# seung-lab/euclidean-distance-transform-3d

Hardware: AMD Instinct MI355X
Metric: Mvox/s edt3dsq 512^3 uint32 (higher is better)
Workload: dtype u16 integer quanta (exact) with f64 envelope fallback / f32 storage / u32 labels; 1 GPU; cfg2: 512^3 uint32 labels, anisotropy (6.0, 6.0, 30.0), black_border=True, device-resident in/out

## Files before the change

### euclidean-distance-transform-3d_amd/csrc/edt_api.hip

```cpp
#include <algorithm>
#include <atomic>
#include <cstdlib>
#include <cstring>
#include <mutex>
#include <system_error>
#include <thread>
#include <vector>

#include <sys/mman.h>

#include "edt_common.h"
#include "edt_kernels.h"

#include "edt_api_internal.h"

namespace edt_amd {

static thread_local std::string g_last_error = "";
#ifdef EDT_DIAG
constexpr int kDiagMask = ~0;
#else
constexpr int kDiagMask = kDiagFormBits;
#endif
static int env_debug_mode() {
// ... 32 lines not shown


struct Plan {
  int ndim;
  int64_t sx, sy, sz, voxels;
  AxisGeom gy, gz;
  float *bufB = nullptr;
  int32_t *stack = nullptr;
  uint32_t *nz_y = nullptr, *rs_y = nullptr, *zs_y = nullptr, *nz_z = nullptr, *rs_z = nullptr;
  unsigned char *line_ws = nullptr;
  uint16_t *codes = nullptr;
  int64_t xy_slab = 0;
  bool codes_whole = false;
  int64_t code_pitch = 0;
  uint32_t *q16_counts = nullptr, *q16_ids = nullptr;
  uint32_t *q16_map = nullptr;
  int q16_map_words = 0;
  int64_t q16_id_capacity = 0;
  size_t bytes = 0;
};

AxisGeom make_geom_y(int64_t sx, int64_t sy, int64_t sz) {
  AxisGeom g;
  g.sx = sx; g.n = sy; g.stride = sx; g.nouter = sz; g.outer_stride = sx * sy;
  g.nbands = ceil_div(sy, kBandRows);
  return g;
}
AxisGeom make_geom_z(int64_t sx, int64_t sy, int64_t sz) {
  AxisGeom g;
  g.sx = sx; g.n = sz; g.stride = sx * sy; g.nouter = sy; g.outer_stride = sx;
  g.nbands = ceil_div(sz, kBandRows);
  return g;
}

static bool plan_needs_pingpong(int ndim, int64_t sx, int64_t sy, int64_t sz, int flags);

constexpr int64_t kCodeSlabVoxels = (int64_t)1 << 27;
static int64_t whole_index_limit() {
  static const int64_t v = [] {
    const char *e = std::getenv("EDT_HIP_WHOLE_INDEX_BYTES");
    return e ? (int64_t)std::strtoll(e, nullptr, 0) : (int64_t)8 << 30;
  }();
  return v;
}
static int64_t plane_pad_elems(int64_t sx, int64_t sy) {
  const char *e = std::getenv("EDT_HIP_PLANE_PAD_BYTES");
  const int64_t forced = (e && *e) ? (int64_t)std::strtoll(e, nullptr, 0) : (int64_t)-1;
  if (forced >= 0) return (forced & ~(int64_t)7) / 2;
  const int64_t slice = sx * sy * (int64_t)sizeof(uint16_t);
  if (slice % ((int64_t)2 << 20) == 0) return 8192 / 2;
  if (slice % ((int64_t)1 << 20) == 0) return 4096 / 2;
  return 0;
}
constexpr int kQ16Slots = 256;
constexpr int EDT_FLAG_NO_INDEX_FORM = 0x8000;
static int64_t plan_code_slab(int dtype, int ndim, int64_t sx, int64_t sy, int64_t sz, int flags) {
  if (ndim < 2 || sx % 4 != 0 || sx * sy > kCodeSlabVoxels || (flags & (EDT_FLAG_NO_INDEX_FORM | EDT_FLAG_SMALL_WORKSPACE))) return 0;
  if ((flags & EDT_FLAG_FORCE_GENERIC) || env_force_generic() || (g_debug_mode & (0x100000 | 64 | 32))) return 0;
  if (!row_pass_wave_supported(dtype, sx, sy, sz) || !column_pass_wave_supported(make_geom_y(sx, sy, sz))) return 0;
  int64_t slab = kCodeSlabVoxels / (sx * sy);
  if (slab >= sz) return sz;
  if (slab >= 32) slab &= ~(int64_t)31;
  return slab;
}

static Plan make_plan(int dtype, int ndim, int64_t sx, int64_t sy, int64_t sz, void *ws, int flags) {
  Plan p;
  p.ndim = ndim; p.sx = sx; p.sy = sy; p.sz = sz; p.voxels = sx * sy * sz;
  p.gy = make_geom_y(sx, sy, sz);
  p.gz = make_geom_z(sx, sy, sz);
  Carver c(ws);
  if (ndim >= 2) {
    if (plan_needs_pingpong(ndim, sx, sy, sz, flags)) {
      p.bufB = c.take<float>((size_t)p.voxels);
      p.stack = c.take<int32_t>((size_t)p.voxels);
    }
    const size_t wy = (size_t)(p.gy.sx * p.gy.nbands * p.gy.nouter);
    p.nz_y = c.take<uint32_t>(wy);
    p.rs_y = c.take<uint32_t>(wy);
  }
  if (ndim >= 3 && !(flags & EDT_FLAG_BATCH_2D)) {
    const size_t wy = (size_t)(p.gy.sx * p.gy.nbands * p.gy.nouter);
    const size_t wz = (size_t)(p.gz.sx * p.gz.nbands * p.gz.nouter);
    p.nz_z = c.take<uint32_t>(wz);
    if (wz <= wy) p.rs_z = p.rs_y;
    else p.rs_z = c.take<uint32_t>(wz);
    p.zs_y = c.take<uint32_t>(wy);
  }
  if (ndim >= 2) {
    p.xy_slab = plan_code_slab(dtype, ndim, sx, sy, sz, flags);
    p.codes_whole = p.xy_slab >= sz || (p.xy_slab > 0 && p.xy_slab % 32 == 0 && ndim == 3 && !(flags & EDT_FLAG_BATCH_2D) &&
                                        sx * sy * sz * (int64_t)sizeof(uint16_t) <= whole_index_limit());
    p.code_pitch = sx * sy + ((p.codes_whole && ndim == 3 && sz > 1 && !(flags & EDT_FLAG_BATCH_2D)) ? plane_pad_elems(sx, sy) : 0);
    if (p.xy_slab > 0) p.codes = c.take<uint16_t>((size_t)((p.codes_whole ? sz : p.xy_slab) * p.code_pitch));
  }
  if (ndim >= 2 && !(flags & EDT_FLAG_FORCE_GENERIC) && !env_force_generic()) {
    const int64_t ty = ceil_div(sx, 16) * (ceil_div(sz, 8) * 8);
    const int64_t tz = ceil_div(sx, 16) * (ceil_div(sy, 8) * 8);
    p.q16_map_words = (int)ceil_div(sz, 32);
    p.q16_counts = c.take<uint32_t>(kQ16Slots + (size_t)(ceil_div(sx, 32) * p.q16_map_words));
    p.q16_map = p.q16_counts ? p.q16_counts + kQ16Slots : nullptr;
    p.q16_id_capacity = std::max(ty, tz);
    p.q16_ids = c.take<uint32_t>((size_t)p.q16_id_capacity);
  }
  if (ndim == 1) (void)c.take<unsigned char>(line_workspace_bytes(sx));
  if (ndim >= 2 && !row_pass_tiled_supported(sx) && !row_pass_wave_supported(dtype, sx, sy, sz) &&
      !(flags & EDT_FLAG_FORCE_GENERIC) && !env_force_generic())
    p.line_ws = c.take<unsigned char>(rows_line_workspace_bytes(sx, sy * sz));
  p.bytes = align_up(c.off, 256) + 256;
  return p;
}

bool column_inplace_supported(const AxisGeom &g) {
  return column_pass_wave_supported(g) || column_pass_tiled_supported(g);
}
int launch_column_inplace(float *F, const uint32_t *nz, const uint32_t *rs, const AxisGeom &g,
// ... 75 lines not shown
                      float wx, float wy, float wz, int flags, float *d_out, void *d_ws,
                      size_t ws_bytes, hipStream_t stream) {
  int rc = check_shape(dtype, ndim, sx, sy, sz);
  if (rc != EDT_OK) return rc;
  if ((rc = check_voxel_sizes(ndim, wx, wy, wz)) != EDT_OK) return rc;
  if (sx == 0 || sy == 0 || sz == 0) return EDT_OK;
  if (!d_labels || !d_out) { set_error("null device pointer"); return EDT_ERR_BAD_ARG; }
  Plan p = make_plan(dtype, ndim, sx, sy, sz, d_ws, flags);
  if (d_ws && ws_bytes < p.bytes && p.codes != nullptr) p = make_plan(dtype, ndim, sx, sy, sz, d_ws, flags | EDT_FLAG_NO_INDEX_FORM);
  const bool line_without_ws = ndim == 1 && (!d_ws || ws_bytes < p.bytes);
  if (!line_without_ws && (!d_ws || ws_bytes < p.bytes)) {
    set_error("workspace too small: need " + std::to_string(p.bytes) +
              " bytes (edt_hip_workspace_bytes_flags with the flags of this call)");
    return EDT_ERR_BAD_ARG;
  }
  const int bb = (flags & EDT_FLAG_BLACK_BORDER) ? 1 : 0;
  const int want_sqrt = (flags & EDT_FLAG_SQRT) ? 1 : 0;
  const int signed_tf = (flags & EDT_FLAG_SIGNED) ? 1 : 0;
  if (signed_tf && !signed_transform_supported(dtype, ndim, sx, sy, sz, flags)) {
    set_error("EDT_FLAG_SIGNED: shape not served by the one-transform form (edt_hip_signed_supported)");
    return EDT_ERR_UNSUPPORTED;
  }
  const int last_epi = (bb ? 0 : kEpiToInf) | (want_sqrt ? kEpiSqrt : 0) | kEpiStream;
  if ((flags & EDT_FLAG_BATCH_2D) && ndim != 3) { set_error("EDT_FLAG_BATCH_2D needs ndim = 3 (sz = image count)"); return EDT_ERR_BAD_ARG; }
  const bool zpass = ndim == 3 && !(flags & EDT_FLAG_BATCH_2D);
  const bool binary_yz = (flags & EDT_FLAG_BINARY_YZ) != 0 && dtype != EDT_BOOL;
  const float fmin_y = edt_hip_field_floor(wx, wx);
  const float fmin_z = edt_hip_field_floor(wx, wy);
  p.gy.fmin = fmin_y;
  p.gz.fmin = fmin_z;

  if (g_log.enabled.load(std::memory_order_relaxed)) {
    std::lock_guard<std::mutex> lock(g_log_mutex);
    log_begin_call();
  }

  float q16_q = 1.0f;
  uint32_t q16_a[3] = {1u, 1u, 1u};
  bool q16 = false;
  int q16_slot = 0;
  bool q16_counts_zeroed = false;
  if (ndim >= 2 && p.q16_counts != nullptr) {
    const float ws3[3] = {wx, wy, wz};
    q16 = q16_quantum(ws3, (ndim == 3 && !(flags & EDT_FLAG_BATCH_2D)) ? 3 : 2, &q16_q, q16_a);
  }
  constexpr int kQ16Off = 16 | 64 | 0x2000 | 0x4000 | 0x8000 | 0x10000;
  auto q16_cannot_refuse = [&](int axis, const AxisGeom &g) {
    return q16 && q16_no_refusals(q16_q, q16_a, axis, sx, sy, g.n, bb);
  };
  auto q16_applies = [&](const AxisGeom &g) {
    return q16 && column_pass_q16_supported(g) && column_pass_wave_supported(g) && !(g_debug_mode & kQ16Off) &&
           ceil_div(g.sx, 16) * (ceil_div(g.nouter, 8) * 8) <= p.q16_id_capacity;
  };
  auto q16_pass = [&](float *F, const uint16_t *codes, const uint32_t *rs, const AxisGeom &g, int axis, int epi,
                      TileList &list, uint16_t *plane, bool sure, bool &launched, int64_t map_words_off = 0,
                      const uint32_t *signbits = nullptr) -> int {
    list = TileList();
    launched = false;
    if (!q16 || q16_slot >= kQ16Slots || !column_pass_q16_supported(g) || !column_pass_wave_supported(g) ||
        !column_pass_q16_aligned(F, codes, plane) || (g_debug_mode & kQ16Off))
      return EDT_OK;
    if (ceil_div(g.sx, 16) * (ceil_div(g.nouter, 8) * 8) > p.q16_id_capacity) return EDT_OK;
    sure = sure && q16_cannot_refuse(axis, g);
    if (!sure && !q16_counts_zeroed) {
      EDT_HIP_TRY(hipMemsetAsync(p.q16_counts, 0, kQ16Slots * sizeof(uint32_t), stream));
      q16_counts_zeroed = true;
    }
    uint32_t *count = p.q16_counts + q16_slot++;
    const bool reads_plane = codes == nullptr && plane != nullptr;
    const int r = launch_column_pass_q16(F, codes, rs, g, q16_q, q16_a[axis], q16_a[0], bb, epi, count, p.q16_ids, stream,
                                         nullptr, plane, p.q16_map + map_words_off, p.q16_map_words, nullptr,
                                         reads_plane ? p.code_pitch : 0, reads_plane ? sx : 0,
                                         (axis == 1 && plane != nullptr && codes != nullptr && q16_value_limit(q16_q, q16_a[2], sz, bb) != 0u) ? 1 : 0,
                                         signbits, (codes != nullptr && axis == 1) ? p.code_pitch : 0);
    if (r != EDT_OK) return r;
    launched = true;
    list.count = count;
    list.ids = p.q16_ids;
    list.none = sure;
    return EDT_OK;
  };

  if (ndim == 1) {
    ScopedPass t("x_pass", stream);
    if (force_generic_1d(flags) || line_without_ws) return launch_row_pass_serial(dtype, d_labels, d_out, sx, 1, wx, bb, 0, want_sqrt, stream);
    return launch_line_pass(dtype, d_labels, d_out, sx, wx, bb, want_sqrt, d_ws, stream);
  }

  const bool force_generic = (flags & EDT_FLAG_FORCE_GENERIC) != 0 || env_force_generic();
  const bool tiled_y = !force_generic && column_inplace_supported(p.gy);
  const bool tiled_z = !force_generic && column_inplace_supported(p.gz);
  const int swaps = (tiled_y ? 0 : 1) + ((zpass && !tiled_z) ? 1 : 0);
  float *cur = (swaps % 2 == 0) ? d_out : p.bufB;
  float *other = (cur == d_out) ? p.bufB : d_out;
  const bool tiled_x = !force_generic && (row_pass_tiled_supported(sx) || row_pass_wave_supported(dtype, sx, sy, sz));
  const bool index_form = p.codes != nullptr && tiled_x && tiled_y && row_codes_exact(wx, sx);
  bool plane16 = q16 && index_form && zpass && p.codes_whole && !(g_debug_mode & (kQ16Off | 0x10000000)) &&
                       column_pass_q16_supported(p.gy) && column_pass_q16_supported(p.gz) &&
                       column_pass_wave_supported(p.gy) && column_pass_wave_supported(p.gz);
  bool y_sure = true;
  const bool q16_only = zpass && index_form && tiled_z && q16_applies(p.gy) && q16_applies(p.gz) && q16_cannot_refuse(1, p.gy) &&
                        q16_cannot_refuse(2, p.gz) && column_pass_q16_aligned(cur, p.codes, p.codes) &&
                        ceil_div(sz, p.xy_slab > 0 ? p.xy_slab : sz) + 1 <= kQ16Slots;
  const bool fuse_sign = signed_tf && q16_only && !(g_debug_mode & 0x400);
  const int zero_label = fuse_sign ? 2 : signed_tf;
  const bool skip_nz = q16_only && !signed_tf && !binary_yz && !(g_debug_mode & 0x400);
  uint32_t *const nzy = skip_nz ? nullptr : p.nz_y, *const nzz = skip_nz ? nullptr : p.nz_z;
  if (index_form) {
    const int64_t sxy = sx * sy, wpl = p.gy.sx * p.gy.nbands;
    const size_t lsz = dtype_size(dtype);
    const bool one = p.xy_slab >= sz;
    ScopedPass whole(one ? nullptr : "xy_pass", stream);
    for (int64_t z0 = 0; z0 < sz; z0 += p.xy_slab) {
      const int64_t zc = std::min<int64_t>(p.xy_slab, sz - z0);
      const char *lab = static_cast<const char *>(d_labels) + (size_t)(z0 * sxy) * lsz;
      uint16_t *slab_codes = p.codes + ((p.codes_whole && !one) ? z0 * p.code_pitch : 0);
      {
        ScopedPass t(one ? "x_pass" : nullptr, stream);
        rc = launch_row_pass_wave(dtype, lab, nullptr, nzy ? nzy + z0 * wpl : nullptr, p.rs_y + z0 * wpl,
                                  zpass ? p.zs_y + z0 * wpl : nullptr, sx, sy, zc, wx, bb, bb ? 0 : 1, stream,
                                  z0 > 0 ? lab - (size_t)sxy * lsz : nullptr, slab_codes, zero_label, p.code_pitch);
        if (rc != EDT_OK) return rc;
        if (binary_yz) {
          AxisGeom gb = p.gy;
          gb.nouter = zc;
          rc = launch_planes_one_run(p.nz_y + z0 * wpl, p.rs_y + z0 * wpl, zpass ? p.zs_y + z0 * wpl : nullptr, gb, z0, stream);
          if (rc != EDT_OK) return rc;
        }
      }
      {
        ScopedPass t(one ? "y_pass" : nullptr, stream);
        AxisGeom g = p.gy;
        g.nouter = zc;
        TileList list;
        bool launched = false;
        rc = q16_pass(cur + z0 * sxy, slab_codes, p.rs_y + z0 * wpl, g, 1, zpass ? 0 : last_epi, list, plane16 ? slab_codes : nullptr,
                      true, launched, (p.codes_whole && !one) ? z0 / 32 : 0);
        if (rc != EDT_OK) return rc;
        if (!launched) plane16 = false;
        y_sure = y_sure && list.none;
        if (q16_only && (!launched || !list.none)) { set_error("internal: pass Y left the integer kernel"); return EDT_ERR_HIP; }
        if (!list.none)
          rc = launch_column_pass_wave_codes(cur + z0 * sxy, slab_codes, p.nz_y + z0 * wpl, p.rs_y + z0 * wpl, g, wy, bb,
                                             zpass ? 0 : last_epi, wx, bb ? 0 : 1, stream, nullptr, list, ColumnOut(), p.code_pitch);
        if (rc != EDT_OK) return rc;
      }
    }
  } else if (tiled_x) {
    {
      ScopedPass t("x_pass", stream);
      if (signed_tf)
        rc = launch_row_pass_wave(dtype, d_labels, cur, p.nz_y, p.rs_y, zpass ? p.zs_y : nullptr, sx, sy, sz, wx, bb, bb ? 0 : 1,
                                  stream, nullptr, nullptr, 1);
      else
        rc = launch_row_bits(dtype, d_labels, cur, p.nz_y, p.rs_y, zpass ? p.zs_y : nullptr, sx, sy, sz,
                             wx, bb, bb ? 0 : 1, stream);
      if (rc != EDT_OK) return rc;
      if (binary_yz) rc = launch_planes_one_run(p.nz_y, p.rs_y, zpass ? p.zs_y : nullptr, p.gy, 0, stream);
      if (rc != EDT_OK) return rc;
    }
  } else {
    {
      ScopedPass t("x_pass", stream);
      if (p.line_ws != nullptr) rc = launch_rows_line_pass(dtype, d_labels, cur, sx, sy * sz, wx, bb, bb ? 0 : 1, p.line_ws, stream);
      else rc = launch_row_pass_serial(dtype, d_labels, cur, sx, sy * sz, wx, bb, bb ? 0 : 1, 0, stream);
      if (rc != EDT_OK) return rc;
    }
    {
      ScopedPass t("y_bits", stream);
      rc = launch_axis_bits(dtype, d_labels, nullptr, p.nz_y, p.rs_y, p.gy, stream);
      if (rc != EDT_OK) return rc;
      if (binary_yz) rc = launch_planes_one_run(p.nz_y, p.rs_y, nullptr, p.gy, 0, stream);
      if (rc != EDT_OK) return rc;
    }
  }
  if (!index_form) {
    ScopedPass t("y_pass", stream);
    const int epi = zpass ? 0 : last_epi;
    if (tiled_y) {
      TileList list;
      bool launched = false;
      rc = q16_pass(cur, nullptr, p.rs_y, p.gy, 1, epi, list, nullptr, false, launched);
      if (rc != EDT_OK) return rc;
      y_sure = false;
      rc = launch_column_inplace(cur, p.nz_y, p.rs_y, p.gy, wy, bb, epi, stream, list);
    } else {
      rc = launch_column_pass_serial(cur, other, p.nz_y, p.rs_y, p.stack, p.gy, wy, bb, epi, stream);
      std::swap(cur, other);
    }
    if (rc != EDT_OK) return rc;
  }
  if (zpass) {
    ScopedPass t("z_bits", stream);
    if (tiled_x) rc = launch_bits_transpose_yz(nzy, p.zs_y, nzz, p.rs_z, sx, sy, sz, stream);
    else {
      rc = launch_axis_bits(dtype, d_labels, nullptr, p.nz_z, p.rs_z, p.gz, stream);
      if (rc == EDT_OK && binary_yz) rc = launch_planes_one_run(p.nz_z, p.rs_z, nullptr, p.gz, 0, stream);
    }
// ... 50 lines not shown
  }
  return n;
}

const char *edt_hip_last_error(void) { return last_error_cstr(); }

int edt_hip_index_form_exact(float wx, int64_t sx) { return (sx >= 1 && row_codes_exact(wx, sx)) ? 1 : 0; }

const char *edt_hip_version(void) { return "edt_hip 0.1 (gfx950)"; }

size_t edt_hip_workspace_bytes_flags(int dtype, int ndim, int64_t sx, int64_t sy, int64_t sz, int flags) {
  if (check_shape(dtype, ndim, sx, sy, sz) != EDT_OK) return 0;
  if (sx == 0 || sy == 0 || sz == 0) return 256;
  return make_plan(dtype, ndim, sx, sy, sz, nullptr, flags).bytes;
}

int edt_hip_signed_supported(int dtype, int ndim, int64_t sx, int64_t sy, int64_t sz, int flags) {
  if (check_shape(dtype, ndim, sx, sy, sz) != EDT_OK) return 0;
  return signed_transform_supported(dtype, ndim, sx, sy, sz, flags) ? 1 : 0;
}

size_t edt_hip_workspace_bytes(int dtype, int ndim, int64_t sx, int64_t sy, int64_t sz) {
  return edt_hip_workspace_bytes_flags(dtype, ndim, sx, sy, sz, 0);
}

int edt_hip_edtsq_device(const void *d_labels, int dtype, int ndim, int64_t sx, int64_t sy,
                         int64_t sz, float wx, float wy, float wz, int flags, float *d_output,
                         void *d_workspace, size_t workspace_bytes, void *stream) {
  return run_device(d_labels, dtype, ndim, sx, sy, sz, wx, wy, wz, flags, d_output, d_workspace,
                    workspace_bytes, (hipStream_t)stream);
}

int edt_hip_set_debug_mode(int mode) {
  set_thread_debug_mode(mode);
  return EDT_OK;
}

int edt_hip_get_debug_mode(void) { return debug_mode(); }

int edt_hip_q16_no_refusals(int64_t sx, int64_t sy, int64_t sz, float wx, float wy, float wz, int ndim, int black_border,
                            int *pass_y, int *pass_z) {
  if (pass_y) *pass_y = 0;
  if (pass_z) *pass_z = 0;
  if (ndim < 2 || ndim > 3 || sx < 1 || sy < 1 || (ndim == 3 && sz < 1)) return 0;
  const float w3[3] = {wx, wy, wz};
  float q = 1.0f;
  uint32_t a[3] = {1u, 1u, 1u};
  if (!q16_quantum(w3, ndim, &q, a)) return 0;
  const bool y = q16_no_refusals(q, a, 1, sx, sy, sy, black_border);
  const bool z = ndim == 3 && y && q16_no_refusals(q, a, 2, sx, sy, sz, black_border);
  if (pass_y) *pass_y = y ? 1 : 0;
  if (pass_z) *pass_z = z ? 1 : 0;
  return 1;
}

int edt_hip_set_profiling(int enabled) {
  std::lock_guard<std::mutex> lock(g_log_mutex);
  g_log.enabled.store(enabled != 0);
  log_begin_call();
  return EDT_OK;
}

int edt_hip_get_pass_times(float *ms, int capacity) {
  std::lock_guard<std::mutex> lock(g_log_mutex);
  int n = (int)g_log.span.size();
  for (int i = 0; i < n && i < capacity; ++i) {
    float t = 0.0f;
    if (hipEventElapsedTime(&t, g_log.pool[g_log.span[i].first], g_log.pool[g_log.span[i].second]) !=
        hipSuccess) {
      (void)hipGetLastError();
      t = -1.0f;
    }
    ms[i] = t;
  }
  return n;
}

const char *edt_hip_get_pass_name(int index) {
  std::lock_guard<std::mutex> lock(g_log_mutex);
  if (index < 0 || index >= (int)g_log.names.size()) return "";
  return g_log.names[index].c_str();
}

float edt_hip_field_floor(float wx, float wy) {
  const float a = wx * wx, b = wy * wy;
  if (!(a > 0.0f) || !(b > 0.0f) || !(a < INFINITY) || !(b < INFINITY)) return 0.0f;
  return a < b ? a : b;
}

int edt_hip_subtract_device(const float *d_a, const float *d_b, float *d_out, int64_t count,
                            void *stream) {
  return launch_subtract(d_a, d_b, d_out, count, (hipStream_t)stream);
}

static bool vg_use_native(int ndim, int64_t sx, int64_t sy, int64_t sz) {
  return !(g_debug_mode & 0x20000) && vg_native_supported(ndim, sx, sy, sz);
}

size_t edt_hip_voxel_graph_workspace_bytes(int ndim, int64_t sx, int64_t sy, int64_t sz) {
  if (check_shape(EDT_U8, ndim, sx, sy, sz) != EDT_OK || ndim < 2) return 0;
  if (sx == 0 || sy == 0 || sz == 0) return 256;
  if (vg_use_native(ndim, sx, sy, sz)) return vg_native_workspace_bytes(ndim, sx, sy, sz);
  const int64_t X = 2 * sx, Y = 2 * sy, Z = (ndim == 3) ? 2 * sz : 1;
  const size_t big = (size_t)(X * Y * Z);
  return align_up(big, 256) + align_up(big * sizeof(float), 256) + edt_hip_workspace_bytes(EDT_U8, ndim, X, Y, Z) + 256;
}
// ... 67 lines not shown
```

### euclidean-distance-transform-3d_amd/csrc/edt_rowwave.hip

```cpp
#include "edt_common.h"
#include "edt_kernels.h"

#include <cmath>

#pragma clang fp contract(off)

#ifndef EDT_ROW_STORE_AUX
#define EDT_ROW_STORE_AUX 0
#endif

namespace edt_amd {

namespace {

constexpr int kRowWaves = 4;

__device__ __forceinline__ void shift_in(uint32_t &w, unsigned long long mask) {
  asm volatile("v_addc_co_u32 %0, vcc, %0, %0, %1" : "+v"(w) : "s"(mask) : "vcc");
}

__device__ __forceinline__ int as_int(float v) { return __float_as_int(v); }

using rsrc_t = __amdgpu_buffer_rsrc_t;
__device__ __forceinline__ rsrc_t make_rsrc(const void *p) {
// ... 214 lines not shown
    }
    {
      const uint32_t poff = (uint32_t)((nrows - 1) * sx) * OB;
#pragma unroll
      for (int c = 0; c < NC; ++c) {
        const int x = xb + c * 64 + lane;
        if (FULL || x < sx) {
          if (C16) __builtin_amdgcn_raw_buffer_store_b16((uint16_t)pend[c], rs_out, (uint32_t)x * 2u, poff, EDT_ROW_STORE_AUX);
          else __builtin_amdgcn_raw_buffer_store_b32((uint32_t)pend[c], rs_out, (uint32_t)x * 4u, poff, EDT_ROW_STORE_AUX);
        }
      }
    }

    const int sh = 32 - nrows;
    const int64_t wbase = ((int64_t)z * nby + yb) * sx;
#pragma unroll
    for (int c = 0; c < NC; ++c) {
      const int x = xb + c * 64 + lane;
      if (FULL || x < sx) {
        const uint32_t ys = (__brev(ysw[c]) >> sh) | (y0 == 0 ? 1u : 0u);
        const uint32_t zs = (z == 0 && halo == nullptr) ? (0xFFFFFFFFu >> sh) : (__brev(zsw[c]) >> sh);
        if (nz_y != nullptr) nz_y[wbase + x] = __brev(nzw[c]) >> sh;
        ys_y[wbase + x] = ys;
        if (HAS_Z) zs_y[wbase + x] = zs;
      }
    }
  }
}

bool row_codes_exact(float w, int64_t sx) {
  if (!(w >= 1.0e-30f) || !(w <= 1.0e30f) || sx + 2 >= 0xFFFF) return false;
  int e = 0;
  const float fr = std::frexp(w, &e);
  uint64_t m = (uint64_t)std::ldexp((double)fr, 24);
  while (m != 0 && !(m & 1u)) m >>= 1;
  if (m * (uint64_t)(sx + 1) >= (1ull << 24)) return false;
  return (double)w * (double)(sx + 1) < 3.0e38;
}

bool row_pass_wave_supported(int dtype, int64_t sx, int64_t sy, int64_t sz) {
  const int64_t widest = (debug_mode() & 0x4000000) ? 1024 : (debug_mode() & 32) ? 2048 : 4096;
  return sx >= 1 && sx <= widest && sy * sz < (int64_t)1 << 30 && sx * sy * sz < ((int64_t)1 << 40);
}

template <typename T, int NC, int H = 1>
static int launch_row_wave_tn(const void *labels, float *out, uint32_t *nz_y, uint32_t *ys_y,
                              uint32_t *zs_y, int64_t sx, int64_t sy, int64_t sz, float w, int bb,
                              int to_finite, hipStream_t stream, const void *halo, bool codes, int zero_label, int64_t opitch) {
  const int64_t nby = ceil_div(sy, kBandRows);
  const int64_t ngroups = nby * sz;
  if (ngroups <= 0) return EDT_OK;
  constexpr int GW = H >= 2 ? 1 : kRowWaves;
  constexpr int WAVES = H >= 2 ? H : kRowWaves;
  const size_t lds = (size_t)(((sx + 3 + 3) & ~(int64_t)3) + 4 * H) * sizeof(float);
  int64_t blocks = ceil_div(ngroups, GW);
  const int64_t resident = 256 * 8 * (kRowWaves / WAVES > 0 ? kRowWaves / WAVES : 1);
  if (blocks > resident) blocks = resident;
  const int xcd_sched = row_xcd_schedule(nby, sz, &blocks, GW, resident / 8);
#define LAUNCH(Z, F, C)                                                                                   \
  hipLaunchKernelGGL((k_row_pass_wave<T, NC, Z, F, C, H>), dim3((unsigned)blocks), dim3(WAVES * 64), lds, stream,  \
                     (const T *)labels, out, nz_y, ys_y, zs_y, (int)sx, (int)sy, (int)sz, w, bb, to_finite, \
                     (int)nby, (int)ngroups, xcd_sched, (const T *)halo, zero_label, opitch)
#define LAUNCH_C(Z, F) do { if (codes) LAUNCH(Z, F, true); else LAUNCH(Z, F, false); } while (0)
  const bool full = sx == 64 * NC * H;
  if (zs_y != nullptr) { if (full) LAUNCH_C(true, true); else LAUNCH_C(true, false); }
  else { if (full) LAUNCH_C(false, true); else LAUNCH_C(false, false); }
#undef LAUNCH_C
#undef LAUNCH
  EDT_HIP_TRY(hipGetLastError());
  return EDT_OK;
}

template <typename T>
static int launch_row_wave_t(const void *labels, float *out, uint32_t *nz_y, uint32_t *ys_y,
                             uint32_t *zs_y, int64_t sx, int64_t sy, int64_t sz, float w, int bb,
                             int to_finite, hipStream_t stream, const void *halo, bool codes, int zero_label, int64_t opitch) {
  const int64_t nc = ceil_div(sx, 64);
#define GO(N) return launch_row_wave_tn<T, N>(labels, out, nz_y, ys_y, zs_y, sx, sy, sz, w, bb, to_finite, stream, halo, codes, zero_label, opitch)
  if (nc <= 1) GO(1);
  if (nc <= 2) GO(2);
  if (nc <= 4) GO(4);
  if (nc <= 8) GO(8);
  if (nc <= 16) GO(16);
#undef GO
#define GO2(N) return launch_row_wave_tn<T, N, 2>(labels, out, nz_y, ys_y, zs_y, sx, sy, sz, w, bb, to_finite, stream, halo, codes, zero_label, opitch)
  if (nc <= 20) GO2(10);
  if (nc <= 24) GO2(12);
  if (nc <= 28) GO2(14);
  if (nc <= 32) GO2(16);
#undef GO2
#define GO4(N) return launch_row_wave_tn<T, N, 4>(labels, out, nz_y, ys_y, zs_y, sx, sy, sz, w, bb, to_finite, stream, halo, codes, zero_label, opitch)
  if (nc <= 48) GO4(12);
  GO4(16);
#undef GO4
}

int launch_row_pass_wave(int dtype, const void *labels, float *out, uint32_t *nz_y, uint32_t *ys_y,
                         uint32_t *zs_y, int64_t sx, int64_t sy, int64_t sz, float w, int bb,
                         int to_finite, hipStream_t stream, const void *halo, uint16_t *codes, int zero_label, int64_t codes_pitch) {
  const int64_t opitch = (codes != nullptr && codes_pitch > 0) ? codes_pitch : sx * sy;
  if (codes != nullptr) out = reinterpret_cast<float *>(codes);
#define ROW_WAVE(T) \
  return launch_row_wave_t<T>(labels, out, nz_y, ys_y, zs_y, sx, sy, sz, w, bb, to_finite, stream, halo, codes != nullptr, zero_label, opitch)
  switch (dtype) {
    case EDT_U8: case EDT_BOOL: ROW_WAVE(uint8_t);
    case EDT_U16: ROW_WAVE(uint16_t);
    case EDT_U32: ROW_WAVE(uint32_t);
// ... 10 lines not shown
```

### euclidean-distance-transform-3d_amd/edt/_lib.py

```python
from __future__ import annotations

import ctypes
import os

_HERE = os.path.dirname(os.path.abspath(__file__))
LIB_PATH = os.environ.get("EDT_HIP_LIB") or os.path.join(os.path.dirname(_HERE), "lib", "libedt_hip.so")

U8, U16, U32, U64, F32, F64, BOOL = range(7)
DTYPE_SIZE = {U8: 1, U16: 2, U32: 4, U64: 8, F32: 4, F64: 8, BOOL: 1}

FLAG_BLACK_BORDER = 1
FLAG_SQRT = 2
FLAG_FORCE_GENERIC = 4
FLAG_BATCH_2D = 8
FLAG_SMALL_WORKSPACE = 16
FLAG_BINARY_YZ = 32
FLAG_SIGNED = 64

OK = 0
ERR_NO_DEVICE = -1


class EdtHipError(RuntimeError):
    def __init__(self, code: int, message: str):
        super().__init__(f"edt_hip error {code}: {message}")
        self.code = code


_vp, _i, _i64, _f, _sz = (ctypes.c_void_p, ctypes.c_int, ctypes.c_int64, ctypes.c_float,
                          ctypes.c_size_t)
_d = ctypes.c_double

SIGNATURES = {
    "edt_hip_device_count": (_i, []),
    "edt_hip_last_error": (ctypes.c_char_p, []),
    "edt_hip_version": (ctypes.c_char_p, []),
    "edt_hip_squared_edt_1d_multi_seg": (_i, [_vp, _i, _vp, _i64, _i64, _f, _i]),
    "edt_hip_edt2dsq": (_i, [_vp, _i, _i64, _i64, _f, _f, _i, _i, _vp]),
    "edt_hip_edt3dsq": (_i, [_vp, _i, _i64, _i64, _i64, _f, _f, _f, _i, _i, _vp]),
    "edt_hip_edt2d": (_i, [_vp, _i, _i64, _i64, _f, _f, _i, _i, _vp]),
    "edt_hip_edt3d": (_i, [_vp, _i, _i64, _i64, _i64, _f, _f, _f, _i, _i, _vp]),
    "edt_hip_edt2dsq_voxel_graph": (_i, [_vp, _i, _vp, _i64, _i64, _f, _f, _i, _vp]),
    "edt_hip_edt3dsq_voxel_graph": (_i, [_vp, _i, _vp, _i64, _i64, _i64, _f, _f, _f, _i, _vp]),
    "edt_hip_binary_edtsq": (_i, [_vp, _i, _i, _i64, _i64, _i64, _f, _f, _f, _i, _i, _vp]),
    "edt_hip_edt2dsq_batch": (_i, [_vp, _i, _i64, _i64, _i64, _f, _f, _i, _i, _vp]),
    "edt_hip_runs_workspace_bytes": (_sz, [_i64]),
    "edt_hip_extract_runs_device": (_i, [_vp, _i, _i64, _vp, _i64, _vp, _vp, _sz, _vp]),
    "edt_hip_edt3dsq_multi": (_i, [_vp, _i, _i64, _i64, _i64, _f, _f, _f, _i, _i, _vp, _vp, _i]),
    "edt_hip_set_devices": (_i, [_vp, _i]),
    "edt_hip_multi_supported": (_i, [_i, _i64, _i64, _i64, _i]),
    "edt_hip_sdf": (_i, [_vp, _i, _i, _i64, _i64, _i64, _f, _f, _f, _i, _i, _vp]),
    "edt_hip_signed_supported": (_i, [_i, _i, _i64, _i64, _i64, _i]),
    "edt_hip_workspace_bytes": (_sz, [_i, _i, _i64, _i64, _i64]),
    "edt_hip_workspace_bytes_flags": (_sz, [_i, _i, _i64, _i64, _i64, _i]),
    "edt_hip_index_form_exact": (_i, [_f, _i64]),
    "edt_hip_edtsq_device": (_i, [_vp, _i, _i, _i64, _i64, _i64, _f, _f, _f, _i, _vp, _vp, _sz, _vp]),
    "edt_hip_set_profiling": (_i, [_i]),
    "edt_hip_set_debug_mode": (_i, [_i]),
    "edt_hip_get_debug_mode": (_i, []),
    "edt_hip_q16_no_refusals": (_i, [_i64, _i64, _i64, _f, _f, _f, _i, _i, _vp, _vp]),
    "edt_hip_release_cache": (_i, []),
    "edt_hip_get_pass_times": (_i, [_vp, _i]),
    "edt_hip_get_pass_name": (ctypes.c_char_p, [_i]),
    "edt_hip_shard_workspace_bytes": (_sz, [_i, _i64, _i64, _i64]),
    "edt_hip_shard_xy_device": (_i, [_vp, _vp, _i, _i64, _i64, _i64, _f, _f, _i, _vp, _vp, _vp, _sz, _vp]),
    "edt_hip_shard_z_device": (_i, [_vp, _vp, _i64, _i64, _i64, _f, _i, _vp, _sz, _vp]),
    "edt_hip_shard_records_supported": (_i, [_i, _i64, _i64, _i64]),
    "edt_hip_shard_record_floats": (_sz, [_i64, _i64]),
    "edt_hip_shard_records_workspace_bytes": (_sz, [_i, _i64, _i64, _i64]),
    "edt_hip_shard_xy_records_device": (_i, [_vp, _vp, _i, _i64, _i64, _i64, _f, _f, _i, _i, _vp, _vp, _vp, _sz, _vp]),
    "edt_hip_shard_z_records_device": (_i, [_vp, _i64, _i64, _i64, _f, _i, _vp, _sz, _vp]),
    "edt_hip_shard_z_device_ex": (_i, [_vp, _vp, _i64, _i64, _i64, _f, _f, _i, _vp, _sz, _vp]),
    "edt_hip_shard_z_records_device_ex": (_i, [_vp, _i64, _i64, _i64, _f, _f, _i, _vp, _sz, _vp]),
    "edt_hip_shard_z_records_device_w": (_i, [_vp, _i64, _i64, _i64, _f, _f, _f, _i, _vp, _sz, _vp]),
    "edt_hip_shard_records16_supported": (_i, [_i, _i64, _i64, _i64, _f, _f, _f]),
    "edt_hip_shard_record16_words": (_sz, [_i64, _i64]),
    "edt_hip_shard_xy_records16_device": (_i, [_vp, _vp, _i, _i64, _i64, _i64, _f, _f, _f, _i, _i, _vp, _vp, _vp, _vp, _sz, _vp]),
    "edt_hip_shard_z_records16_device": (_i, [_vp, _vp, _i64, _i64, _i64, _f, _f, _f, _i, _vp, _sz, _vp]),
    "edt_hip_field_floor": (_f, [_f, _f]),
    "edt_hip_subtract_device": (_i, [_vp, _vp, _vp, _i64, _vp]),
    "edt_hip_voxel_graph_workspace_bytes": (_sz, [_i, _i64, _i64, _i64]),
    "edt_hip_edtsq_voxel_graph_device": (_i, [_vp, _i, _vp, _i, _i64, _i64, _i64, _f, _f, _f, _i, _vp, _vp, _sz, _vp]),
    "edt_hip_select_label_device": (_i, [_vp, _i, _vp, _vp, _vp, _i64, _vp]),
    "edt_hip_is_background_device": (_i, [_vp, _i, _vp, _i64, _vp]),
    "edt_hip_feature_workspace_bytes": (_sz, [_i, _i, _i64, _i64, _i64, _i]),
    "edt_hip_feature_transform_device": (_i, [_vp, _i, _i, _i64, _i64, _i64, _f, _f, _f, _i, _vp, _vp, _sz, _vp]),
    "edt_hip_feature_transform": (_i, [_vp, _i, _i, _i64, _i64, _i64, _f, _f, _f, _i, _vp]),
    "edt_hip_expand_labels_workspace_bytes": (_sz, [_i, _i, _i64, _i64, _i64]),
    "edt_hip_expand_labels_device": (_i, [_vp, _i, _i, _i64, _i64, _i64, _f, _f, _f, _d, _vp, _vp, _sz, _vp]),
    "edt_hip_expand_labels": (_i, [_vp, _i, _i, _i64, _i64, _i64, _f, _f, _f, _d, _vp]),
    "edt_hip_label_stats_workspace_bytes": (_sz, [_i, _i64, _i64]),
    "edt_hip_label_stats_device": (_i, [_vp, _i, _vp, _i, _i64, _i64, _i64, _i64, _vp, _vp, _vp, _vp, _vp, _vp, _vp, _sz, _vp]),
    "edt_hip_label_stats": (_i, [_vp, _i, _i, _i64, _i64, _i64, _f, _f, _f, _i, _vp, _i64, _vp, _vp, _vp, _vp, _vp, _vp]),
}

_lib = None


def _preload_hip_runtime() -> None:
    import importlib.util
    import sys
    if "torch" in sys.modules:
        return
    try:
        spec = importlib.util.find_spec("torch")
    except (ImportError, ValueError):
        spec = None
    if spec is None or not spec.origin:
        return
    cand = os.path.join(os.path.dirname(spec.origin), "lib", "libamdhip64.so")
    if os.path.exists(cand):
        try:
            ctypes.CDLL(cand, mode=ctypes.RTLD_GLOBAL)
# ... 43 lines not shown
```

### include/edt_hip.h

```cpp
#ifndef EDT_HIP_H
#define EDT_HIP_H

#include <stddef.h>
#include <stdint.h>

#ifdef __cplusplus
extern "C" {
#endif

enum {
  EDT_U8 = 0,
  EDT_U16 = 1,
  EDT_U32 = 2,
  EDT_U64 = 3,
  EDT_F32 = 4,
  EDT_F64 = 5,
  EDT_BOOL = 6
};

enum {
  EDT_OK = 0,
  EDT_ERR_NO_DEVICE = -1,
  EDT_ERR_BAD_ARG = -2,
  EDT_ERR_HIP = -3,
// ... 19 lines not shown


int edt_hip_squared_edt_1d_multi_seg(const void *labels, int dtype, float *dest, int64_t n,
                                     int64_t stride, float anisotropy, int black_border);

int edt_hip_edt2dsq(const void *labels, int dtype, int64_t sx, int64_t sy, float wx, float wy,
                    int black_border, int parallel, float *output);

int edt_hip_edt3dsq(const void *labels, int dtype, int64_t sx, int64_t sy, int64_t sz, float wx,
                    float wy, float wz, int black_border, int parallel, float *output);

int edt_hip_edt2d(const void *labels, int dtype, int64_t sx, int64_t sy, float wx, float wy,
                  int black_border, int parallel, float *output);
int edt_hip_edt3d(const void *labels, int dtype, int64_t sx, int64_t sy, int64_t sz, float wx,
                  float wy, float wz, int black_border, int parallel, float *output);

int edt_hip_edt2dsq_voxel_graph(const void *labels, int dtype, const uint8_t *graph, int64_t sx,
                                int64_t sy, float wx, float wy, int black_border,
                                float *workspace);
int edt_hip_edt3dsq_voxel_graph(const void *labels, int dtype, const uint8_t *graph, int64_t sx,
                                int64_t sy, int64_t sz, float wx, float wy, float wz,
                                int black_border, float *workspace);

int edt_hip_binary_edtsq(const void *labels, int dtype, int ndim, int64_t sx, int64_t sy, int64_t sz, float wx,
                         float wy, float wz, int black_border, int take_sqrt, float *output);

int edt_hip_edt3dsq_multi(const void *labels, int dtype, int64_t sx, int64_t sy, int64_t sz, float wx, float wy,
                          float wz, int black_border, int take_sqrt, float *output, const int *devices,
                          int n_devices);
int edt_hip_multi_supported(int dtype, int64_t sx, int64_t sy, int64_t sz, int n_devices);
int edt_hip_set_devices(const int *devices, int n_devices);

int edt_hip_sdf(const void *labels, int dtype, int ndim, int64_t sx, int64_t sy, int64_t sz, float wx, float wy,
                float wz, int black_border, int squared, float *output);

int edt_hip_release_cache(void);


size_t edt_hip_workspace_bytes(int dtype, int ndim, int64_t sx, int64_t sy, int64_t sz);
size_t edt_hip_workspace_bytes_flags(int dtype, int ndim, int64_t sx, int64_t sy, int64_t sz, int flags);

int edt_hip_edt2dsq_batch(const void *labels, int dtype, int64_t sx, int64_t sy, int64_t count, float wx, float wy,
                          int black_border, int take_sqrt, float *output);

int edt_hip_edtsq_device(const void *d_labels, int dtype, int ndim, int64_t sx, int64_t sy,
                         int64_t sz, float wx, float wy, float wz, int flags, float *d_output,
                         void *d_workspace, size_t workspace_bytes, void *stream);

int edt_hip_set_profiling(int enabled);
int edt_hip_set_debug_mode(int mode);
int edt_hip_get_debug_mode(void);
int edt_hip_q16_no_refusals(int64_t sx, int64_t sy, int64_t sz, float wx, float wy, float wz, int ndim, int black_border,
                            int *pass_y, int *pass_z);
int edt_hip_get_pass_times(float *ms, int capacity);
const char *edt_hip_get_pass_name(int index);

size_t edt_hip_shard_workspace_bytes(int dtype, int64_t sx, int64_t sy, int64_t sz);
int edt_hip_shard_xy_device(const void *d_labels, const void *d_halo, int dtype, int64_t sx,
                            int64_t sy, int64_t sz_local, float wx, float wy, int flags,
                            float *d_partial, uint8_t *d_zflags, void *d_workspace,
                            size_t workspace_bytes, void *stream);
int edt_hip_shard_z_device(float *d_partial, const uint8_t *d_zflags, int64_t sx,
                           int64_t sy_local, int64_t sz, float wz, int flags,
                           void *d_workspace, size_t workspace_bytes, void *stream);
float edt_hip_field_floor(float wx, float wy);
int edt_hip_shard_z_device_ex(float *d_partial, const uint8_t *d_zflags, int64_t sx,
                              int64_t sy_local, int64_t sz, float wz, float field_floor, int flags,
                              void *d_workspace, size_t workspace_bytes, void *stream);

int edt_hip_shard_records_supported(int dtype, int64_t sx, int64_t sy, int64_t sz);
size_t edt_hip_shard_record_floats(int64_t sx, int64_t y_rows);
size_t edt_hip_shard_records_workspace_bytes(int dtype, int64_t sx, int64_t sy, int64_t sz);
int edt_hip_shard_xy_records_device(const void *d_labels, const void *d_halo, int dtype, int64_t sx,
                                    int64_t sy, int64_t sz_local, float wx, float wy, int flags,
                                    int nparts, const int64_t *y_splits, void *const *d_blocks,
                                    void *d_workspace, size_t workspace_bytes, void *stream);
int edt_hip_shard_z_records_device(float *d_records, int64_t sx, int64_t sy_local, int64_t sz,
                                   float wz, int flags, void *d_workspace, size_t workspace_bytes,
                                   void *stream);
int edt_hip_shard_z_records_device_ex(float *d_records, int64_t sx, int64_t sy_local, int64_t sz,
                                      float wz, float field_floor, int flags, void *d_workspace,
                                      size_t workspace_bytes, void *stream);
int edt_hip_shard_z_records_device_w(float *d_records, int64_t sx, int64_t sy_local, int64_t sz, float wx, float wy,
                                     float wz, int flags, void *d_workspace, size_t workspace_bytes, void *stream);

int edt_hip_shard_records16_supported(int dtype, int64_t sx, int64_t sy, int64_t sz, float wx, float wy, float wz);
size_t edt_hip_shard_record16_words(int64_t sx, int64_t y_rows);
int edt_hip_shard_xy_records16_device(const void *d_labels, const void *d_halo, int dtype, int64_t sx, int64_t sy,
                                      int64_t sz_local, float wx, float wy, float wz, int flags, int nparts,
                                      const int64_t *y_splits, void *const *d_blocks, uint32_t *d_refused, void *d_workspace,
                                      size_t workspace_bytes, void *stream);
int edt_hip_shard_z_records16_device(const void *d_records, float *d_out, int64_t sx, int64_t sy_local, int64_t sz, float wx,
                                     float wy, float wz, int flags, void *d_workspace, size_t workspace_bytes, void *stream);

int edt_hip_subtract_device(const float *d_a, const float *d_b, float *d_out, int64_t count,
                            void *stream);
size_t edt_hip_runs_workspace_bytes(int64_t count);
int edt_hip_extract_runs_device(const void *d_labels, int dtype, int64_t count, int64_t *d_starts, int64_t capacity,
                                int64_t *d_count, void *d_workspace, size_t workspace_bytes, void *stream);

int edt_hip_is_background_device(const void *d_labels, int dtype, uint8_t *d_mask, int64_t count,
                                 void *stream);

size_t edt_hip_voxel_graph_workspace_bytes(int ndim, int64_t sx, int64_t sy, int64_t sz);
int edt_hip_edtsq_voxel_graph_device(const void *d_labels, int dtype, const uint8_t *d_graph, int ndim,
                                     int64_t sx, int64_t sy, int64_t sz, float wx, float wy, float wz,
// ... 36 lines not shown
```

Baseline: 249,400 Mvox/s.

## Add optional side-stream overlap of XY slab passes and drop unused row-pass LDS

Adds an env-gated path that splits the XY stage into z-slabs. The Y column pass of each slab runs on a side stream, ordered with a ring of events, so it can overlap the X row pass of the next slab. A separate env budget can shrink the code slab size so that more slabs exist to pipeline. The row-wave launch also stops reserving dynamic LDS when it emits codes with H==1, which may allow more resident blocks. By default the budget is zero and overlap is off, and a 512^3 volume fits in one slab, so only the LDS change takes effect. The overlap path adds event synchronisation and stream-ordering risk on the q16 counters.

```diff
diff --git a/euclidean-distance-transform-3d_amd/csrc/edt_api.hip b/euclidean-distance-transform-3d_amd/csrc/edt_api.hip
--- a/euclidean-distance-transform-3d_amd/csrc/edt_api.hip
+++ b/euclidean-distance-transform-3d_amd/csrc/edt_api.hip
@@ -108,6 +108,11 @@
   if (slice % ((int64_t)1 << 20) == 0) return 4096 / 2;
   return 0;
 }
+constexpr int64_t kXYSlabBytesDefault = 0;
+static int64_t xy_slab_budget() {
+  const char *e = std::getenv("EDT_HIP_XY_SLAB_BYTES");
+  return (e && *e) ? (int64_t)std::strtoll(e, nullptr, 0) : kXYSlabBytesDefault;
+}
 constexpr int kQ16Slots = 256;
 constexpr int EDT_FLAG_NO_INDEX_FORM = 0x8000;
 static int64_t plan_code_slab(int dtype, int ndim, int64_t sx, int64_t sy, int64_t sz, int flags) {
@@ -115,9 +120,54 @@
   if ((flags & EDT_FLAG_FORCE_GENERIC) || env_force_generic() || (g_debug_mode & (0x100000 | 64 | 32))) return 0;
   if (!row_pass_wave_supported(dtype, sx, sy, sz) || !column_pass_wave_supported(make_geom_y(sx, sy, sz))) return 0;
   int64_t slab = kCodeSlabVoxels / (sx * sy);
-  if (slab >= sz) return sz;
-  if (slab >= 32) slab &= ~(int64_t)31;
-  return slab;
+  if (slab >= sz) slab = sz;
+  else if (slab >= 32) slab &= ~(int64_t)31;
+  const int64_t budget = xy_slab_budget();
+  if (budget <= 0 || sz <= 32 || slab < 32) return slab;
+  const int64_t slice8 = sx * sy * ((int64_t)dtype_size(dtype) * 8 + 16 + 3);
+  int64_t cut = std::max<int64_t>(32, (std::min(budget, (int64_t)1 << 56) * 8 / slice8) & ~(int64_t)31);
+  cut = std::max(cut, (ceil_div(sz, (int64_t)kQ16Slots - 1) + 31) & ~(int64_t)31);
+  if (cut >= slab) return slab;
+  const bool stack2d = ndim == 3 && (flags & EDT_FLAG_BATCH_2D);
+  if (!stack2d && sx * sy * sz * (int64_t)sizeof(uint16_t) > whole_index_limit()) return slab;
+  return cut;
+}
+
+struct XYFork {
+  static constexpr int kRing = 4;
+  int device = -1;
+  hipStream_t side = nullptr;
+  hipEvent_t x_done[kRing] = {}, y_done[kRing] = {};
+};
+static bool xy_overlap_enabled() {
+  const char *e = std::getenv("EDT_HIP_XY_OVERLAP");
+  return e && e[0] == '1';
+}
+static XYFork *xy_fork_for(hipStream_t s) {
+  hipStreamCaptureStatus cap = hipStreamCaptureStatusNone;
+  if (hipStreamIsCapturing(s, &cap) != hipSuccess || cap != hipStreamCaptureStatusNone) {
+    (void)hipGetLastError();
+    return nullptr;
+  }
+  int dev = -1;
+  if (hipGetDevice(&dev) != hipSuccess) { (void)hipGetLastError(); return nullptr; }
+  static thread_local std::vector<XYFork *> forks;
+  for (XYFork *f : forks)
+    if (f->device == dev) return f->side ? f : nullptr;
+  XYFork *f = new XYFork;
+  f->device = dev;
+  forks.push_back(f);
+  bool ok = hipStreamCreateWithFlags(&f->side, hipStreamNonBlocking) == hipSuccess;
+  for (int i = 0; ok && i < XYFork::kRing; ++i)
+    ok = hipEventCreateWithFlags(&f->x_done[i], hipEventDisableTiming) == hipSuccess &&
+         hipEventCreateWithFlags(&f->y_done[i], hipEventDisableTiming) == hipSuccess;
+  if (!ok) {
+    (void)hipGetLastError();
+    if (f->side) (void)hipStreamDestroy(f->side);
+    f->side = nullptr;
+    return nullptr;
+  }
+  return f;
 }
 
 static Plan make_plan(int dtype, int ndim, int64_t sx, int64_t sy, int64_t sz, void *ws, int flags) {
@@ -299,6 +349,7 @@
     return q16 && column_pass_q16_supported(g) && column_pass_wave_supported(g) && !(g_debug_mode & kQ16Off) &&
            ceil_div(g.sx, 16) * (ceil_div(g.nouter, 8) * 8) <= p.q16_id_capacity;
   };
+  hipStream_t col_stream = stream;
   auto q16_pass = [&](float *F, const uint16_t *codes, const uint32_t *rs, const AxisGeom &g, int axis, int epi,
                       TileList &list, uint16_t *plane, bool sure, bool &launched, int64_t map_words_off = 0,
                       const uint32_t *signbits = nullptr) -> int {
@@ -310,12 +361,12 @@
     if (ceil_div(g.sx, 16) * (ceil_div(g.nouter, 8) * 8) > p.q16_id_capacity) return EDT_OK;
     sure = sure && q16_cannot_refuse(axis, g);
     if (!sure && !q16_counts_zeroed) {
-      EDT_HIP_TRY(hipMemsetAsync(p.q16_counts, 0, kQ16Slots * sizeof(uint32_t), stream));
+      EDT_HIP_TRY(hipMemsetAsync(p.q16_counts, 0, kQ16Slots * sizeof(uint32_t), col_stream));
       q16_counts_zeroed = true;
     }
     uint32_t *count = p.q16_counts + q16_slot++;
     const bool reads_plane = codes == nullptr && plane != nullptr;
-    const int r = launch_column_pass_q16(F, codes, rs, g, q16_q, q16_a[axis], q16_a[0], bb, epi, count, p.q16_ids, stream,
+    const int r = launch_column_pass_q16(F, codes, rs, g, q16_q, q16_a[axis], q16_a[0], bb, epi, count, p.q16_ids, col_stream,
                                          nullptr, plane, p.q16_map + map_words_off, p.q16_map_words, nullptr,
                                          reads_plane ? p.code_pitch : 0, reads_plane ? sx : 0,
                                          (axis == 1 && plane != nullptr && codes != nullptr && q16_value_limit(q16_q, q16_a[2], sz, bb) != 0u) ? 1 : 0,
@@ -357,9 +408,26 @@
     const int64_t sxy = sx * sy, wpl = p.gy.sx * p.gy.nbands;
     const size_t lsz = dtype_size(dtype);
     const bool one = p.xy_slab >= sz;
+    XYFork *const fork = (!one && p.codes_whole && xy_overlap_enabled()) ? xy_fork_for(stream) : nullptr;
+    struct Join {
+      XYFork *f; hipStream_t s; int last = -1;
+      bool pending = false;
+      ~Join() {
+        if (!f) return;
+        if (pending && hipEventRecord(f->y_done[(last + 1) % XYFork::kRing], f->side) == hipSuccess) ++last;
+        if (last >= 0) (void)hipStreamWaitEvent(s, f->y_done[last % XYFork::kRing], 0);
+      }
+    };
     ScopedPass whole(one ? nullptr : "xy_pass", stream);
-    for (int64_t z0 = 0; z0 < sz; z0 += p.xy_slab) {
+    Join join{fork, stream};
+    if (fork && q16 && !q16_cannot_refuse(1, p.gy) && !q16_counts_zeroed) {
+      EDT_HIP_TRY(hipMemsetAsync(p.q16_counts, 0, kQ16Slots * sizeof(uint32_t), stream));
+      q16_counts_zeroed = true;
+    }
+    int k = 0;
+    for (int64_t z0 = 0; z0 < sz; z0 += p.xy_slab, ++k) {
       const int64_t zc = std::min<int64_t>(p.xy_slab, sz - z0);
+      if (fork && k >= 2) EDT_HIP_TRY(hipStreamWaitEvent(stream, fork->y_done[(k - 2) % XYFork::kRing], 0));
       const char *lab = static_cast<const char *>(d_labels) + (size_t)(z0 * sxy) * lsz;
       uint16_t *slab_codes = p.codes + ((p.codes_whole && !one) ? z0 * p.code_pitch : 0);
       {
@@ -381,6 +449,12 @@
         g.nouter = zc;
         TileList list;
         bool launched = false;
+        if (fork) {
+          EDT_HIP_TRY(hipEventRecord(fork->x_done[k % XYFork::kRing], stream));
+          EDT_HIP_TRY(hipStreamWaitEvent(fork->side, fork->x_done[k % XYFork::kRing], 0));
+        }
+        struct Restore { hipStream_t &ref, v; ~Restore() { ref = v; } } restore{col_stream, stream};
+        if (fork) { col_stream = fork->side; join.pending = true; }
         rc = q16_pass(cur + z0 * sxy, slab_codes, p.rs_y + z0 * wpl, g, 1, zpass ? 0 : last_epi, list, plane16 ? slab_codes : nullptr,
                       true, launched, (p.codes_whole && !one) ? z0 / 32 : 0);
         if (rc != EDT_OK) return rc;
@@ -389,8 +463,13 @@
         if (q16_only && (!launched || !list.none)) { set_error("internal: pass Y left the integer kernel"); return EDT_ERR_HIP; }
         if (!list.none)
           rc = launch_column_pass_wave_codes(cur + z0 * sxy, slab_codes, p.nz_y + z0 * wpl, p.rs_y + z0 * wpl, g, wy, bb,
-                                             zpass ? 0 : last_epi, wx, bb ? 0 : 1, stream, nullptr, list, ColumnOut(), p.code_pitch);
+                                             zpass ? 0 : last_epi, wx, bb ? 0 : 1, col_stream, nullptr, list, ColumnOut(), p.code_pitch);
         if (rc != EDT_OK) return rc;
+        if (fork) {
+          EDT_HIP_TRY(hipEventRecord(fork->y_done[k % XYFork::kRing], fork->side));
+          join.last = k;
+          join.pending = false;
+        }
       }
     }
   } else if (tiled_x) {
@@ -547,6 +626,11 @@
   if (pass_y) *pass_y = y ? 1 : 0;
   if (pass_z) *pass_z = z ? 1 : 0;
   return 1;
+}
+
+int64_t edt_hip_xy_slab_slices(int dtype, int ndim, int64_t sx, int64_t sy, int64_t sz, int flags) {
+  if (check_shape(dtype, ndim, sx, sy, sz) != EDT_OK || sx == 0 || sy == 0 || sz == 0) return 0;
+  return plan_code_slab(dtype, ndim, sx, sy, sz, flags);
 }
 
 int edt_hip_set_profiling(int enabled) {
diff --git a/euclidean-distance-transform-3d_amd/csrc/edt_rowwave.hip b/euclidean-distance-transform-3d_amd/csrc/edt_rowwave.hip
--- a/euclidean-distance-transform-3d_amd/csrc/edt_rowwave.hip
+++ b/euclidean-distance-transform-3d_amd/csrc/edt_rowwave.hip
@@ -290,7 +290,7 @@
   if (ngroups <= 0) return EDT_OK;
   constexpr int GW = H >= 2 ? 1 : kRowWaves;
   constexpr int WAVES = H >= 2 ? H : kRowWaves;
-  const size_t lds = (size_t)(((sx + 3 + 3) & ~(int64_t)3) + 4 * H) * sizeof(float);
+  const size_t lds = (codes && H == 1) ? 0 : (size_t)(((sx + 3 + 3) & ~(int64_t)3) + 4 * H) * sizeof(float);
   int64_t blocks = ceil_div(ngroups, GW);
   const int64_t resident = 256 * 8 * (kRowWaves / WAVES > 0 ? kRowWaves / WAVES : 1);
   if (blocks > resident) blocks = resident;
diff --git a/euclidean-distance-transform-3d_amd/edt/_lib.py b/euclidean-distance-transform-3d_amd/edt/_lib.py
--- a/euclidean-distance-transform-3d_amd/edt/_lib.py
+++ b/euclidean-distance-transform-3d_amd/edt/_lib.py
@@ -59,6 +59,7 @@
     "edt_hip_set_debug_mode": (_i, [_i]),
     "edt_hip_get_debug_mode": (_i, []),
     "edt_hip_q16_no_refusals": (_i, [_i64, _i64, _i64, _f, _f, _f, _i, _i, _vp, _vp]),
+    "edt_hip_xy_slab_slices": (_i64, [_i, _i, _i64, _i64, _i64, _i]),
     "edt_hip_release_cache": (_i, []),
     "edt_hip_get_pass_times": (_i, [_vp, _i]),
     "edt_hip_get_pass_name": (ctypes.c_char_p, [_i]),
diff --git a/include/edt_hip.h b/include/edt_hip.h
--- a/include/edt_hip.h
+++ b/include/edt_hip.h
@@ -95,6 +95,7 @@
 int edt_hip_get_debug_mode(void);
 int edt_hip_q16_no_refusals(int64_t sx, int64_t sy, int64_t sz, float wx, float wy, float wz, int ndim, int black_border,
                             int *pass_y, int *pass_z);
+int64_t edt_hip_xy_slab_slices(int dtype, int ndim, int64_t sx, int64_t sy, int64_t sz, int flags);
 int edt_hip_get_pass_times(float *ms, int capacity);
 const char *edt_hip_get_pass_name(int index);
 
```

Measured after the change: 249,000 Mvox/s. Within noise of the previous version (-0.2%).
